# zyhbili/Dual-Space-NeRF

Hardware: AMD Instinct MI355X
Metric: rendered rays/sec (64 samples/ray), 512x512 frame (higher is better)
Workload: dtype split-f16x3 (3 x v_mfma_f32_32x32x16_f16 on hi/lo fp16 operand halves, f32 accumulate: f32-equivalent accuracy - parity bars of the tests: 1e-4 absolute on RGB / acc / weights against the reference; sigma 1e-4 absolute where |sigma| <= 100 and 4e-6 RELATIVE to max|sigma| above (this checkpoint: |sig

## Files before the change

### dual-space-nerf_amd/csrc/dsn_api.hip

```cpp
#include "../../include/dsnerf.h"
#include "dsn_common.h"
#include "dsn_kernels.h"
#include <cstdlib>

#include <stdio.h>
#include <string.h>

static thread_local char g_err[512] = "";

static int dsn_fail(const char* fmt, const char* a = "", long long b = 0) {
    snprintf(g_err, sizeof(g_err), fmt, a, b);
    return 1;
}
static int dsn_check_launch(const char* what) {
    hipError_t e = hipGetLastError();
    if (e != hipSuccess) { snprintf(g_err, sizeof(g_err), "%s: launch failed: %s", what, hipGetErrorString(e)); return 1; }
    return 0;
}
#define DSN_REQUIRE(cond, msg) do { if (!(cond)) return dsn_fail("%s", msg); } while (0)

thread_local int g_dsn_persistent_override = 0;
namespace {
struct DsnShareCus {
    explicit DsnShareCus(bool on) {
// ... 642 lines not shown
        int32_t *counts = nullptr, *outside0 = nullptr;
        dsn_nn_cellmajor_begin(w.nn_small, &counts, &outside0, st);
        dsn_launch_sample_gg(s.xyz, (flags & DSN_SAMPLE_UNIFORM) ? 0 : V, ray_o, ray_d, near, far, R, S, t_vals, jitter, z, nullptr, st,
                             s.nn_world.fine.g, (int32_t*)w.grad, counts, outside0, (int32_t*)w.grad + N);
        if (lazy) dsn_launch_build_nn_visited(s.cent_world, F, s.nn_world, counts, st);
    } else
        dsn_launch_sample_gg(s.xyz, (flags & DSN_SAMPLE_UNIFORM) ? 0 : V, ray_o, ray_d, near, far, R, S, t_vals, jitter, z, nullptr, st);
    if (skip) {
        if (hipMemsetAsync(w.count, 0, DSN_CNT_BYTES, st) != hipSuccess) return dsn_fail("%s", "dsn_render_rays: memset failed");
    }
    if (cellmajor) {
        int32_t* g3 = (int32_t*)w.grad;
        if (!fused_nn) {
            dsn_launch_nn_cellmajor(s.nn_world, nullptr, ray_o, ray_d, z, N, S, g3, w.sort_scratch, g3 + N, w.nn_small, st);
            dsn_launch_warp(s, nullptr, ray_o, ray_d, z, N, S, nullptr, nullptr, nullptr, w.transparent, w.x_c, nullptr, list, cnt, exh, st,
                            g3 + N, skip);
        } else {
            int32_t* outside = nullptr;
            dsn_launch_nn_cellmajor_warp(s.nn_world, ray_o, ray_d, z, N, S, g3, w.sort_scratch, w.nn_small, s.face_world, s.face_canon,
                                         w.transparent, w.x_c, list, cnt, skip, &outside, st, true, lazy);
            dsn_launch_warp(s, nullptr, ray_o, ray_d, z, N, S, nullptr, nullptr, nullptr, w.transparent, w.x_c, nullptr, list, cnt, exh, st,
                            nullptr, skip, g3, outside);
        }
    } else
        dsn_launch_warp(s, nullptr, ray_o, ray_d, z, N, S, nullptr, nullptr, nullptr, w.transparent, w.x_c, nullptr, list, cnt, exh, st,
                        nullptr, skip);
    if (skip) {
        if (hipMemsetAsync(w.sigma, 0, sizeof(float) * N, st) != hipSuccess)
            return dsn_fail("%s", "dsn_render_rays: memset failed");
    }
    }
    if (do_field) {
    int32_t* const fcnt = skip ? w.count + DSN_CNT_FLAGGED : nullptr;
    if (flags & DSN_FIELD_FP32)
        dsn_launch_field((const float*)packed, s.frame, w.x_c, N, list, cnt, w.sigma, w.essence, w.grad, st);
    else if (skip && (flags & DSN_EARLY_STOP)) {
        const bool screen = (flags & DSN_DENSITY_SCREEN) != 0;
        const bool audit = screen && (flags & DSN_SCREEN_AUDIT);
        int32_t* pcnt = w.count + DSN_CNT_POS;
        dsn_launch_slice_bucket(w.active, w.count + DSN_CNT_ACTIVE, N, S, R, bounds, K, w.slices, w.count + DSN_CNT_SLICE, st);
        dsn_launch_slice_T_init(w.T, R, st);
        static const bool adv_env_ray = [] { const char* e = getenv("DSN_STOP_ADVANCE"); return !(e && e[0] == 'l'); }();
        const bool adv_per_ray = adv_env_ray || custom_schedule;
        const float* scal = (const float*)packed + OFF_SCAL;
        for (int k = 0; k < K; ++k) {
            const int s0 = bounds[k], s1 = bounds[k + 1];
            const int64_t Nk = (int64_t)R * (s1 - s0);
            const int32_t* sl = w.slices + (int64_t)R * s0;
            const int32_t* sc = w.count + DSN_CNT_SLICE + k;
            if (k > 0) {
                int32_t* acnt = w.count + DSN_CNT_ALIVE_K + k;
                if (adv_per_ray) dsn_launch_advance_T(w.sigma, w.transparent, z, ray_d, R, S, bounds[k - 1], s0, k, w.T, st);
                dsn_launch_slice_alive(sl, sc, Nk, S, L, k, w.T, w.sigma, w.transparent, z, ray_d, scal, w.alive, acnt, w.count + DSN_CNT_STOP, st,
                                       adv_per_ray);
                sl = w.alive;
                sc = acnt;
            }
            if (screen) {
                int32_t* kcnt = w.count + DSN_CNT_KEEP_K + k;
                dsn_launch_screen16((const float*)packed, s.frame, w.x_c, Nk, sl, sc, w.sigma, w.keep, kcnt, nullptr, nullptr, st,
                                    audit ? w.audit : nullptr, audit ? w.count + DSN_CNT_AUDIT : nullptr, w.audit_cap);
                sl = w.keep;
                sc = kcnt;
            }
            dsn_launch_field16_fwd((const float*)packed, s.frame, w.x_c, Nk, sl, sc, w.sigma, w.essence, w.masks, w.pos, pcnt, st,
                                   w.rec_cap, fcnt);
            (void)s0;
        }
        float* wq = w.n_w;
        dsn_launch_composite(nullptr, w.sigma, w.transparent, z, ray_d, nullptr, R, S, nullptr, nullptr, nullptr, wq, nullptr, st);
        int32_t* sel = w.alive;
        int32_t* lit = w.slices;
        dsn_launch_cull_lit(w.pos, pcnt, N, w.rec_cap, wq, w.sigma, S, scal, sel, w.count + DSN_CNT_SEL, lit, w.count + DSN_CNT_LIT,
                            w.count + DSN_CNT_STOP + 1, w.colour, st);
        dsn_launch_field16_bwd((const float*)packed, s.frame, w.x_c, N, w.pos, pcnt, w.grad, w.masks, st, w.sigma, w.rec_cap, sel,
                               w.count + DSN_CNT_SEL, fcnt);
        if (w.rec_cap < N)
            dsn_launch_field16_from((const float*)packed, s.frame, w.x_c, N, w.pos, pcnt, w.rec_cap, w.sigma, w.essence, w.grad, st, fcnt);
        dsn_launch_field_fix((const float*)packed, s.frame, w.x_c, N, w.pos, pcnt, w.sigma, w.essence, w.grad, st, fcnt);
        if (audit) dsn_launch_screen_audit(w.audit, w.count + DSN_CNT_AUDIT, w.audit_cap, w.sigma, w.count + DSN_CNT_AUDIT + 4, st);
        list = lit;
        cnt = w.count + DSN_CNT_LIT;
    } else if (skip) {
        int32_t* pcnt = w.count + DSN_CNT_POS;
        const bool screen = (flags & DSN_DENSITY_SCREEN) != 0;
        const bool audit = screen && (flags & DSN_SCREEN_AUDIT);
        if (screen) {
            int32_t* kcnt = w.count + DSN_CNT_KEEP;
            dsn_launch_screen16((const float*)packed, s.frame, w.x_c, N, list, cnt, w.sigma, w.keep, kcnt, nullptr, nullptr, st,
                                audit ? w.audit : nullptr, audit ? w.count + DSN_CNT_AUDIT : nullptr, w.audit_cap);
            list = w.keep;
            cnt = kcnt;
        }
        dsn_launch_field16_fwd((const float*)packed, s.frame, w.x_c, N, list, cnt, w.sigma, w.essence, w.masks, w.pos, pcnt, st,
                               w.rec_cap, fcnt);
        dsn_launch_field16_bwd((const float*)packed, s.frame, w.x_c, N, w.pos, pcnt, w.grad, w.masks, st, w.sigma, w.rec_cap, nullptr, nullptr,
                               fcnt);
        list = w.pos;
        cnt = pcnt;
        if (w.rec_cap < N)
            dsn_launch_field16_from((const float*)packed, s.frame, w.x_c, N, list, cnt, w.rec_cap, w.sigma, w.essence, w.grad, st, fcnt);
        dsn_launch_field_fix((const float*)packed, s.frame, w.x_c, N, list, cnt, w.sigma, w.essence, w.grad, st, fcnt);
        if (audit) dsn_launch_screen_audit(w.audit, w.count + DSN_CNT_AUDIT, w.audit_cap, w.sigma, w.count + DSN_CNT_AUDIT + 4, st);
    } else {
        dsn_launch_field16((const float*)packed, s.frame, w.x_c, N, list, cnt, w.sigma, w.essence, w.grad, st);
        dsn_launch_field_fix((const float*)packed, s.frame, w.x_c, N, list, cnt, w.sigma, w.essence, w.grad, st);
    }
    }
    if (!(flags & DSN_FIELD_FP32) && skip) {
        if (flags & DSN_EARLY_STOP) { list = w.slices; cnt = w.count + DSN_CNT_LIT; }
        else { list = w.pos; cnt = w.count + DSN_CNT_POS; }
    }
    if (do_shade && sweep) {
    int32_t n_sh = 0;
    if (hipMemcpyAsync(&n_sh, cnt, sizeof(int32_t), hipMemcpyDeviceToHost, st) != hipSuccess || hipStreamSynchronize(st) != hipSuccess)
        return dsn_fail("%s", "dsn_render_rays_lights: reading the shading list's length failed");
    const size_t per_light = sizeof(float) * 3 * (size_t)n_sh;
    const int G = per_light == 0 ? sweep->n_lights : (int)std::min<size_t>((size_t)sweep->n_lights, sweep->scratch_bytes / per_light);
    if (G < 1)
        return dsn_fail("dsn_render_rays_lights: light_scratch is too small%s: one light's colours need %lld bytes "
                        "(dsn_render_lights_scratch_bytes)", "", (long long)per_light);
    int32_t* slot = w.alive;
    if (!dsn_composite_multi_supported(S, z, w.sigma, out_weights, slot, w.transparent))
        return dsn_fail("%s", "dsn_render_rays_lights: unaligned arrays for the 16-lane compositor");
    dsn_launch_normal(s, w.x_c, w.grad, N, list, cnt, nullptr, w.n_w, exh, st);
    if (hipMemsetAsync(slot, 0xff, sizeof(int32_t) * (size_t)N, st) != hipSuccess)
        return dsn_fail("%s", "dsn_render_rays_lights: memset failed");
    dsn_launch_slot_map(list, cnt, n_sh, slot, st);
// ... 111 lines not shown
```

### dual-space-nerf_amd/csrc/dsn_field16.hip

```cpp
#include "dsn_common.h"
#include "dsn_kernels.h"

typedef float f32x16 __attribute__((ext_vector_type(16)));
typedef _Float16 half8 __attribute__((ext_vector_type(8)));
#define MFMA16(a, b, c) __builtin_amdgcn_mfma_f32_32x32x16_f16((a), (b), (c), 0, 0, 0)

#if !defined(DSN_EXPERIMENTS) && (defined(F16_ABL) || defined(F16_SABL) || defined(F16_TIMING) || defined(F16_TRAIN_ABL))
#error "F16_ABL / F16_SABL / F16_TIMING are experiment switches (wrong results / debug counters): build with -DDSN_EXPERIMENTS"
#endif
#ifndef F16_SINCOS_OCML
#define F16_SINCOS_OCML 0
#endif
#ifndef F16_FENCE
#define F16_FENCE 0
#endif
#ifndef F16_SGB
#define F16_SGB 1
#endif
#ifndef F16_SGB_VALU
#define F16_SGB_VALU 4
#endif
#ifndef F16_SGB_DS
#define F16_SGB_DS 0
#endif
#ifndef F16_MIX
#define F16_MIX 1
#endif
#ifndef F16_PIPE_LATE
#define F16_PIPE_LATE 1
#endif
#ifndef F16_ABL
#define F16_ABL 0
#endif
#ifndef F16_NEXT_POINT
#define F16_NEXT_POINT 1
#endif
#ifndef F16_DMA_SPREAD
#define F16_DMA_SPREAD 1
#endif
#ifndef F16_BIAS_AHEAD
#define F16_BIAS_AHEAD 1
#endif
#ifndef F16_TIMING
#define F16_TIMING 0
#endif
#ifndef F16_PREFETCH
#define F16_PREFETCH 1
#endif

#define F16_THREADS 256
#if defined(DSN_EXPERIMENTS) && defined(F16_TRAIN_ABL) && (F16_TRAIN_ABL & 32)
#define F16_ST_M(m) (1024 * (m))
#else
#define F16_ST_M(m) (32 * (m))
#endif
#define F16_CHUNK 8
#define F16_RING_SLOTS (2 * F16_CHUNK)
#define F16_NCHUNK (DSN_STREAM_BLOCKS / F16_CHUNK)
#define F16_RANGE 65000.0f
#define F16_GSCALE 0.015625f
#define F16_GUNSCALE 64.0f

#if F16_TIMING
__device__ unsigned long long g_f16_timing[16];
#define F16_STAMP(i) do { if (MODE == F16_FWD) { asm volatile("s_waitcnt vmcnt(0) lgkmcnt(0)" ::: "memory"); tstamp[i] = __builtin_readcyclecounter(); rstamp[i] = wall_clock64(); } } while (0)
extern "C" __attribute__((visibility("default"))) int dsn_debug_timing(unsigned long long* out16, int reset) {
    if (out16 && hipMemcpyFromSymbol(out16, HIP_SYMBOL(g_f16_timing), sizeof(unsigned long long) * 16) != hipSuccess) return 1;
    if (reset) { unsigned long long z[16] = {0}; if (hipMemcpyToSymbol(HIP_SYMBOL(g_f16_timing), z, sizeof(z)) != hipSuccess) return 1; }
    return 0;
}
#else
#define F16_STAMP(i) do { } while (0)
#endif
struct W16 {
    const char* g;
    char* ring;
    unsigned ring_off;
    int wave;
    int nchunk = F16_NCHUNK;
    bool spread = F16_DMA_SPREAD != 0;
    half8 h0, l0, h1, l1;
};

#ifndef F16_POS_OFFS
#define F16_POS_OFFS 0
#endif
__device__ __forceinline__ void w16_stage(const W16& w, int c) {
    const char* src = w.g + (size_t)c * 32768;
    const unsigned dst = w.ring_off + (c & 1) * 32768 + w.wave * 8192 + 4096;
#if F16_POS_OFFS
    asm volatile("s_mov_b32 m0, %1\n\ts_nop 0\n\t"
                 "global_load_lds_dwordx4 %0, off\n\tglobal_load_lds_dwordx4 %0, off offset:1024\n\t"
                 "global_load_lds_dwordx4 %0, off offset:2048\n\tglobal_load_lds_dwordx4 %0, off offset:3072"
                 : : "v"(src - 4096), "s"(dst - 4096) : "memory", "m0");
    asm volatile("s_mov_b32 m0, %1\n\ts_nop 0\n\t"
                 "global_load_lds_dwordx4 %0, off\n\tglobal_load_lds_dwordx4 %0, off offset:1024\n\t"
                 "global_load_lds_dwordx4 %0, off offset:2048\n\tglobal_load_lds_dwordx4 %0, off offset:3072"
                 : : "v"(src), "s"(dst) : "memory", "m0");
    return;
#endif
    asm volatile("s_mov_b32 m0, %1\n\ts_nop 0\n\t"
                 "global_load_lds_dwordx4 %0, off offset:-4096\n\tglobal_load_lds_dwordx4 %0, off offset:-3072\n\t"
                 "global_load_lds_dwordx4 %0, off offset:-2048\n\tglobal_load_lds_dwordx4 %0, off offset:-1024\n\t"
                 "global_load_lds_dwordx4 %0, off\n\tglobal_load_lds_dwordx4 %0, off offset:1024\n\t"
                 "global_load_lds_dwordx4 %0, off offset:2048\n\tglobal_load_lds_dwordx4 %0, off offset:3072"
                 : : "v"(src), "s"(dst) : "memory", "m0");
}
template <int I>
__device__ __forceinline__ void w16_stage_part(const W16& w, int c) {
    const char* src = w.g + (size_t)c * 32768;
    const unsigned dst = w.ring_off + (c & 1) * 32768 + w.wave * 8192 + 4096;
#if F16_POS_OFFS
    {
        const int back = I < 2 ? 4096 : 0;
        asm volatile("s_mov_b32 m0, %1\n\ts_nop 0\n\t"
                     "global_load_lds_dwordx4 %0, off offset:%2\n\tglobal_load_lds_dwordx4 %0, off offset:%3"
                     : : "v"(src - back), "s"(dst - back), "n"(2048 * (I & 1)), "n"(2048 * (I & 1) + 1024) : "memory", "m0");
        return;
    }
#endif
    asm volatile("s_mov_b32 m0, %1\n\ts_nop 0\n\t"
                 "global_load_lds_dwordx4 %0, off offset:%2\n\tglobal_load_lds_dwordx4 %0, off offset:%3"
                 : : "v"(src), "s"(dst), "n"(-4096 + 2048 * I), "n"(-3072 + 2048 * I) : "memory", "m0");
}
__device__ __forceinline__ void w16_boundary(const W16& w, int b) {
#if !(F16_ABL & 2)
    asm volatile("s_waitcnt vmcnt(0)" ::: "memory");
#endif
#if !(F16_ABL & 1)
    __syncthreads();
#endif
    const int c = b / F16_CHUNK;
#if !(F16_ABL & 4)
    if (!w.spread && c + 1 < w.nchunk) w16_stage(w, c + 1);
#endif
}
__device__ __forceinline__ void w16_read(const W16& w, int b, int lane, half8& h0, half8& l0, half8& h1, half8& l1) {
    const char* s = w.ring + ((b >> 3) & 1) * 32768 + (b & 7) * 1024 + lane * 16;
    h0 = *reinterpret_cast<const half8*>(s);
    l0 = *reinterpret_cast<const half8*>(s + 8192);
    h1 = *reinterpret_cast<const half8*>(s + 16384);
    l1 = *reinterpret_cast<const half8*>(s + 24576);
}
__device__ __forceinline__ void w16_begin_issue(W16& w, int first_blk) { w16_stage(w, first_blk / F16_CHUNK); }
__device__ __forceinline__ void w16_begin_wait(W16& w, int lane, int first_blk) {
    w16_boundary(w, first_blk);
#if !(F16_ABL & 4)
    if (w.spread && first_blk / F16_CHUNK + 1 < w.nchunk) w16_stage_part<0>(w, first_blk / F16_CHUNK + 1);
#endif
    w16_read(w, first_blk, lane, w.h0, w.l0, w.h1, w.l1);
}
__device__ __forceinline__ void w16_begin(W16& w, int lane, int first_blk) {
    w16_begin_issue(w, first_blk);
    w16_begin_wait(w, lane, first_blk);
}

struct NoHook { __device__ __forceinline__ void operator()(int) const {} };

template <int KB, bool XLS, class Hook = NoHook>
__device__ __forceinline__ void dense16(W16& w, int& blk, int lane, const half8 (&xh)[KB][2], const half8 (&xl)[KB][2],
                                        f32x16& accM, f32x16& accC, Hook&& hook = NoHook()) {
#pragma unroll
    for (int kb = 0; kb < KB; ++kb) {
#if F16_PREFETCH
        half8 n0 = w.h0, m0 = w.l0, n1 = w.h1, m1 = w.l1;
        if (blk + 1 < DSN_STREAM_BLOCKS) {
            if (((blk + 1) & (F16_CHUNK - 1)) == 0) w16_boundary(w, blk + 1);
#if !(F16_ABL & 4)
            if (w.spread) {
                const int pos = (blk + 1) & (F16_CHUNK - 1), cn = (blk + 1) / F16_CHUNK + 1;
                if (cn < w.nchunk) {
                    if (pos == 0) w16_stage_part<0>(w, cn);
                    if (pos == 1) w16_stage_part<1>(w, cn);
                    if (pos == 2) w16_stage_part<2>(w, cn);
                    if (pos == 3) w16_stage_part<3>(w, cn);
                }
            }
#endif
            w16_read(w, blk + 1, lane, n0, m0, n1, m1);
        }
#else
        if (blk > 0) {
            if ((blk & (F16_CHUNK - 1)) == 0) w16_boundary(w, blk);
            w16_read(w, blk, lane, w.h0, w.l0, w.h1, w.l1);
        }
#endif
        if (XLS) {
            accM = MFMA16(w.h0, xh[kb][0], accM);
            accC = MFMA16(w.h0, xl[kb][0], accC);
            accC = MFMA16(w.l0, xh[kb][0], accC);
            accM = MFMA16(w.h1, xh[kb][1], accM);
            accC = MFMA16(w.h1, xl[kb][1], accC);
            accC = MFMA16(w.l1, xh[kb][1], accC);
        } else {
            accM = MFMA16(w.h0, xh[kb][0], accM);
            accC = MFMA16(w.l0, xh[kb][0], accC);
            accM = MFMA16(w.h0, xl[kb][0], accM);
            accC = MFMA16(w.h1, xh[kb][1], accC);
            accM = MFMA16(w.l1, xh[kb][1], accM);
            accC = MFMA16(w.h1, xl[kb][1], accC);
        }
#if !(F16_ABL & 8)
        hook(kb);
#endif
// ... 281 lines not shown
    }
}
template <bool ST = false>
__device__ __forceinline__ void layer16_bwd(W16& w, int& blk, int lane, const half8 (&xh)[8][2],
                                            const half8 (&xl)[8][2], half8 (&yh)[8][2], half8 (&yl)[8][2],
                                            const uint32_t (&mk)[4], float& ovf, float* st = nullptr, float stscale = F16_GUNSCALE) {
    f32x16 pM = zero16(), pC = zero16();
    uint32_t dummy = 0;
#pragma unroll
    for (int m = 0; m < 8; ++m) {
        f32x16 aM = zero16(), aC = zero16();
        const uint32_t mw = m > 0 ? ((mk[(m - 1) >> 1] >> (16 * ((m - 1) & 1))) & 0xffffu) : 0u;
        if (m == 0) dense16<8, true>(w, blk, lane, xh, xl, aM, aC);
        else dense16<8, true>(w, blk, lane, xh, xl, aM, aC, [&](int kb) { epi_slice<false, ST>(pM, pC, kb, mw, dummy, yh[m - 1], yl[m - 1], ovf, (ST && st) ? st + F16_ST_M(m - 1) : nullptr, stscale); });
        pM = aM; pC = aC;
    }
    const uint32_t mw = (mk[3] >> 16) & 0xffffu;
#pragma unroll
    for (int kb = 0; kb < 8; ++kb) epi_slice<false, ST>(pM, pC, kb, mw, dummy, yh[7], yl[7], ovf, (ST && st) ? st + F16_ST_M(7) : nullptr, stscale);
}

#define F16_FULL 0
#define F16_FWD 1
#define F16_BWD 2
#define F16_TRAIN 3
#define F16_FIRST_BWD_BLOCK (OFF_L6T / DSN_BLK)
template <int MODE>
__global__ void __launch_bounds__(F16_THREADS, 1)
k_field16(const float* __restrict__ packed, const DsnFrameState* __restrict__ fs, const float* __restrict__ x_c,
          int64_t N, const int32_t* __restrict__ active_list, const int32_t* __restrict__ active_count,
          float* __restrict__ sigma, float* __restrict__ essence, float* __restrict__ grad,
          uint4* __restrict__ masks, int32_t* __restrict__ pos_list, int32_t* __restrict__ pos_count,
          float* __restrict__ tr_h, float* __restrict__ tr_a, float* __restrict__ tr_rr, int64_t slot_base, int64_t rec_cap,
          const int32_t* __restrict__ sel, int32_t* __restrict__ flag_count) {
    constexpr bool ST = MODE == F16_TRAIN;
    __shared__ __attribute__((aligned(16))) char ring[F16_RING_SLOTS * 4096];
    __shared__ uint32_t s_mask[7][4][F16_THREADS];
    __shared__ __attribute__((aligned(16))) float s_vec[256 + 2304 + 8];
    __shared__ __attribute__((aligned(16))) half8 s_pe[8][F16_THREADS];
    __shared__ int s_app[8];
#ifndef F16_SHARE_SIMD
    DSN_OWN_SIMD();
#endif
    const int tid0 = threadIdx.x;
    const int lane0 = threadIdx.x & 63;
    const int wave = __builtin_amdgcn_readfirstlane(threadIdx.x >> 6);
    int64_t count = (active_list ? (int64_t)(*active_count) : N) - slot_base;
    if (MODE == F16_BWD && count > rec_cap) count = rec_cap;
    const int64_t ntiles = (count + 127) / 128;
    if ((int64_t)blockIdx.x >= ntiles) return;
    for (int i = tid0; i < 256 + 2304 + 8; i += F16_THREADS)
        s_vec[i] = i < 256 ? fs->bias0[i] : (i < 2560 ? packed[OFF_B1 + (i - 256)] : packed[OFF_SCAL + (i - 2560)]);
    for (int i = tid0; i < 256 + (OFF_WDEN - OFF_B1); i += F16_THREADS) s_vec[i] *= F16_FWD_SCALE;
    const float* const v_bias0 = s_vec;
    const float* const v_b1 = s_vec + 256;
    const float* const v_brgb1 = s_vec + 256 + (OFF_BRGB1 - OFF_B1);
    const float* const v_wden = s_vec + 256 + (OFF_WDEN - OFF_B1);
    const float* const v_wrgb3 = s_vec + 256 + (OFF_WRGB3 - OFF_B1);
    const float* const v_scal = s_vec + 2560;
    W16 w;
    w.g = reinterpret_cast<const char*>(packed + OFF16_BASE) + wave * 8192 + 4096 + lane0 * 16;
    w.ring = ring;
    w.ring_off = (unsigned)(uintptr_t)(__attribute__((address_space(3))) char*)ring;
    w.wave = wave;
    if (MODE == F16_FWD) w.nchunk = F16_FIRST_BWD_BLOCK / F16_CHUNK;
    if (MODE == F16_TRAIN) w.spread = false;
    auto tile_point = [&](int64_t t, bool& ok, int64_t& ls) -> int64_t {
        int64_t sl = (t * 4 + wave) * 32 + (lane0 & 31);
        ok = sl < count;
        if (!ok) sl = count - 1;
        ls = sel ? (int64_t)sel[sl] : slot_base + sl;
        return active_list ? (int64_t)active_list[ls] : ls;
    };
    bool valid_n;
    int64_t lslot_n;
    int64_t pt_n = tile_point(blockIdx.x, valid_n, lslot_n);
    float xn[3] = {x_c[3 * pt_n], x_c[3 * pt_n + 1], x_c[3 * pt_n + 2]};
  for (int64_t tile = blockIdx.x; tile < ntiles; tile += gridDim.x) {
    int tid = tid0, lane = lane0;
    asm volatile("" : "+v"(tid), "+v"(lane), "+v"(w.g));
    const int half = lane >> 5;
#if F16_TIMING
    unsigned long long tstamp[6], rstamp[6];
#endif
    F16_STAMP(0);
    w16_begin_issue(w, MODE == F16_BWD ? F16_FIRST_BWD_BLOCK : 0);
#if !F16_NEXT_POINT
    if (tile != (int64_t)blockIdx.x) { pt_n = tile_point(tile, valid_n, lslot_n); xn[0] = x_c[3 * pt_n]; xn[1] = x_c[3 * pt_n + 1]; xn[2] = x_c[3 * pt_n + 2]; }
#endif
    const bool valid = valid_n;
    const int64_t lslot = lslot_n, pt = pt_n;
    const float xa[3] = {xn[0], xn[1], xn[2]};
    const bool more = F16_NEXT_POINT && MODE != F16_TRAIN && tile + gridDim.x < ntiles;
    if (more) pt_n = tile_point(tile + gridDim.x, valid_n, lslot_n);
#define NEXT_POINT() do { if (more) { xn[0] = x_c[3 * pt_n]; xn[1] = x_c[3 * pt_n + 1]; xn[2] = x_c[3 * pt_n + 2]; } } while (0)
    w16_begin_wait(w, lane, MODE == F16_BWD ? F16_FIRST_BWD_BLOCK : 0);
    int blk = MODE == F16_BWD ? F16_FIRST_BWD_BLOCK : 0;
    F16_STAMP(1);

#define MK_STORE(L, mk) { s_mask[L][0][tid] = mk[0]; s_mask[L][1][tid] = mk[1]; s_mask[L][2][tid] = mk[2]; s_mask[L][3][tid] = mk[3]; }
#define MK_LOAD(L, mk) { mk[0] = s_mask[L][0][tid]; mk[1] = s_mask[L][1][tid]; mk[2] = s_mask[L][2][tid]; mk[3] = s_mask[L][3][tid]; }
    uint32_t mk[4];
    half8 ah[8][2], al[8][2], bh[8][2], bl[8][2];
    float ovf = 0.0f;
    uint4* mrec = masks ? masks + ((size_t)(MODE == F16_BWD ? lslot : pt) * 2 + half) * 7 : nullptr;
    const int64_t tr_ls = N * 256;
#if defined(DSN_EXPERIMENTS) && defined(F16_TRAIN_ABL)
    const int64_t pt_st = (F16_TRAIN_ABL & 8) ? (pt & 4095) : ((F16_TRAIN_ABL & 16) ? (pt & 255) : pt);
    const int64_t sl_st = (tile * 4 + wave) * 32 + (lane & 31);
    const int64_t row_off = (F16_TRAIN_ABL & 32) ? (sl_st >> 5) * 8192 + (sl_st & 31) * 32 : pt_st * 256;
    float* const th = ST && valid && !(F16_TRAIN_ABL & 1) ? tr_h + row_off + 4 * half : nullptr;
    float* const ta = ST && valid && !(F16_TRAIN_ABL & 2) ? tr_a + row_off + 4 * half : nullptr;
#else
    float* const th = ST && valid ? tr_h + pt * 256 + 4 * half : nullptr;
    float* const ta = ST && valid ? tr_a + pt * 256 + 4 * half : nullptr;
#endif

  if (MODE != F16_BWD) {
    half8 ph[2][2], pl[2][2];
    {
        f32x16 pe[2];
#pragma unroll
        for (int t = 0; t < 30; ++t) {
            float s, c;
#if F16_SINCOS_OCML
            sincosf(xa[t % 3] * (float)(1 << (t / 3)), &s, &c);
#else
            dsn_sincos(xa[t % 3] * (float)(1 << (t / 3)), s, c);
#endif
// ... 44 lines not shown
        }
        f32x16 v = unscale16(aM, aC);
        const uint32_t bits = relu_bits16(v);
        if (m & 1) mk[m >> 1] |= bits << 16; else mk[m >> 1] = bits;
        if (ST) store16(th ? th + 4 * tr_ls + F16_ST_M(m) : nullptr, v, 1.0f);
        track16(ovf, v);
        split16<false>(v, ah[m], al[m]);
    }
    MK_STORE(4, mk)
    layer16_fwd<ST>(w, blk, lane, v_b1 + 4 * 256, ah, al, bh, bl, mk, ovf, th ? th + 5 * tr_ls : nullptr); MK_STORE(5, mk)
    float sg_part = 0.0f;
#pragma unroll
    for (int m = 0; m < 8; ++m) {
        f32x16 aM = rows16(v_b1 + 5 * 256, m, half), aC = zero16();
        dense16<8, false>(w, blk, lane, bh, bl, aM, aC);
        f32x16 v = unscale16(aM, aC);
        const uint32_t bits = relu_bits16(v);
        if (m & 1) mk[m >> 1] |= bits << 16; else mk[m >> 1] = bits;
        if (ST) store16(th ? th + 6 * tr_ls + F16_ST_M(m) : nullptr, v, 1.0f);
        const f32x16 wd = rows16(v_wden, m, half);
#pragma unroll
        for (int r = 0; r < 16; ++r) sg_part = fmaf(wd[r], v[r], sg_part);
        track16(ovf, v);
        split16<false>(v, ah[m], al[m]);
    }
#endif
    F16_STAMP(3);
    sg_part += __shfl_xor(sg_part, 32);
    const float sg = sg_part + v_scal[0];
    const bool flag_fwd = !(fmaxf(ovf, __shfl_xor(ovf, 32)) < F16_RANGE);
    if (valid && half == 0) sigma[pt] = flag_fwd ? dsn_nan_flag() : sg;
    if (MODE != F16_TRAIN && flag_fwd && valid && half == 0 && flag_count) atomicAdd(flag_count, 1);
    bool write_rec = ST && valid;
    if (MODE == F16_FWD) {
        const bool pos = valid && half == 0 && (sg > 0.0f || flag_fwd);
        const unsigned long long bm = __ballot(pos);
        const int cnt = __popcll(bm);
        if (lane == 0) s_app[wave] = cnt;
        __syncthreads();
        if (tid == 0) {
            const int tot = s_app[0] + s_app[1] + s_app[2] + s_app[3];
            s_app[4] = tot ? atomicAdd(pos_count, tot) : 0;
        }
        __syncthreads();
        int base = s_app[4];
        for (int k = 0; k < wave; ++k) base += s_app[k];
        const int my = base + __popcll(bm & ((1ull << lane) - 1ull));
        if (pos) pos_list[my] = (int32_t)pt;
        const int rslot = __shfl(my, lane & 31);
        write_rec = ((bm >> (lane & 31)) & 1ull) != 0 && (int64_t)rslot < rec_cap;
        mrec = masks + ((size_t)rslot * 2 + half) * 7;
    }
    if (MODE == F16_FWD || MODE == F16_TRAIN) {
        MK_STORE(6, mk)
        if (write_rec) {
#pragma unroll
            for (int L = 0; L < 7; ++L)
                mrec[L] = make_uint4(s_mask[L][0][tid], s_mask[L][1][tid], s_mask[L][2][tid], s_mask[L][3][tid]);
        }
    }
    {
        float e0 = 0.f, e1 = 0.f, e2 = 0.f;
#pragma unroll
        for (int m = 0; m < 4; ++m) {
            f32x16 aM = rows16(v_brgb1, m, half), aC = zero16();
            dense16<8, false>(w, blk, lane, ah, al, aM, aC);
            const f32x16 v = unscale16(aM, aC);
            const f32x16 w0 = rows16(v_wrgb3 + 0 * 128, m, half);
            const f32x16 w1 = rows16(v_wrgb3 + 1 * 128, m, half);
            const f32x16 w2 = rows16(v_wrgb3 + 2 * 128, m, half);
            if (ST && valid) {
                f32x16 xr;
#pragma unroll
                for (int r = 0; r < 16; ++r) xr[r] = fmaxf(v[r], 0.0f);
                store16(tr_rr + pt * 128 + 4 * half + 32 * m, xr, 1.0f);
            }
#pragma unroll
            for (int r = 0; r < 16; ++r) {
                const float x = fmaxf(v[r], 0.0f);
                e0 = fmaf(w0[r], x, e0); e1 = fmaf(w1[r], x, e1); e2 = fmaf(w2[r], x, e2);
            }
        }
        e0 += __shfl_xor(e0, 32); e1 += __shfl_xor(e1, 32); e2 += __shfl_xor(e2, 32);
        if (valid && half == 0) {
            essence[3 * pt + 0] = e0 + v_scal[1];
            essence[3 * pt + 1] = e1 + v_scal[2];
            essence[3 * pt + 2] = e2 + v_scal[3];
        }
    }

#if F16_TIMING
    F16_STAMP(4);
    if (MODE == F16_FWD && tid == 0) {
        for (int i = 0; i < 4; ++i) { atomicAdd(&g_f16_timing[i], tstamp[i + 1] - tstamp[i]); atomicAdd(&g_f16_timing[8 + i], rstamp[i + 1] - rstamp[i]); }
        atomicAdd(&g_f16_timing[7], 1ull);
    }
#endif
    if (MODE == F16_FWD) { __syncthreads(); continue; }
  } else {
#pragma unroll
    for (int L = 0; L < 7; ++L) {
        const uint4 q = mrec[L];
        s_mask[L][0][tid] = q.x; s_mask[L][1][tid] = q.y; s_mask[L][2][tid] = q.z; s_mask[L][3][tid] = q.w;
    }
    MK_LOAD(6, mk)
  }

#pragma unroll
    for (int m = 0; m < 8; ++m) {
        f32x16 g = rows16(v_wden, m, half);
#pragma unroll
        for (int r = 0; r < 16; ++r) g[r] *= F16_GSCALE;
        mask16(g, (mk[m >> 1] >> (16 * (m & 1))) & 0xffffu);
        if (ST) store16(ta ? ta + 6 * tr_ls + F16_ST_M(m) : nullptr, g, F16_GUNSCALE);
        split16<true>(g, ah[m], al[m]);
    }
    MK_LOAD(5, mk) layer16_bwd<ST>(w, blk, lane, ah, al, bh, bl, mk, ovf, ta ? ta + 5 * tr_ls : nullptr);
    if (MODE == F16_BWD) NEXT_POINT();
    MK_LOAD(4, mk) layer16_bwd<ST>(w, blk, lane, bh, bl, ah, al, mk, ovf, ta ? ta + 4 * tr_ls : nullptr);
    MK_LOAD(3, mk)
    f32x16 dpe[2];
#pragma unroll
    for (int m = 0; m < 8; ++m) {
        f32x16 aM = zero16(), aC = zero16();
        dense16<8, true>(w, blk, lane, ah, al, aM, aC);
        f32x16 v = fold16(aM, aC);
        mask16(v, (mk[m >> 1] >> (16 * (m & 1))) & 0xffffu);
        if (ST) store16(ta ? ta + 3 * tr_ls + F16_ST_M(m) : nullptr, v, F16_GUNSCALE);
        track16(ovf, v);
        split16<true>(v, bh[m], bl[m]);
    }
// ... 15 lines not shown
        for (int r = 0; r < 16; ++r) dpe[b][r] += v[r];
    }

    {
        float xb[3] = {xa[0], xa[1], xa[2]};
        asm volatile("" : "+v"(xb[0]), "+v"(xb[1]), "+v"(xb[2]));
        float g[3] = {0.f, 0.f, 0.f};
#pragma unroll
        for (int t = 0; t < 30; ++t) {
            const int j = t / 3, a = t % 3;
            float s, c;
#if F16_SINCOS_OCML
            sincosf(xb[a] * (float)(1 << j), &s, &c);
#else
            dsn_sincos(xb[a] * (float)(1 << j), s, c);
#endif
            const float d = dpe[t >> 4][t & 15];
            const float term = (d * (half ? s : c)) * (float)(1 << j);
            g[a] += half ? -term : term;
        }
        const float i30 = dpe[1][14], i31 = dpe[1][15];
        if (half) g[1] += i30; else { g[0] += i30; g[2] += i31; }
        g[0] += __shfl_xor(g[0], 32); g[1] += __shfl_xor(g[1], 32); g[2] += __shfl_xor(g[2], 32);
        if (valid && half == 0) {
            grad[3 * pt] = g[0] * F16_GUNSCALE; grad[3 * pt + 1] = g[1] * F16_GUNSCALE; grad[3 * pt + 2] = g[2] * F16_GUNSCALE;
        }
    }
    const bool flagged = !(fmaxf(ovf, __shfl_xor(ovf, 32)) < F16_RANGE);
    if (flagged && valid && half == 0) {
        if (MODE == F16_TRAIN) { if (pos_count) atomicAdd(pos_count, 1); }
        else { sigma[pt] = dsn_nan_flag(); if (flag_count) atomicAdd(flag_count, 1); }
    }
    if (MODE == F16_TRAIN) break;
    __syncthreads();
  }
}

void dsn_launch_field16(const float* packed, const DsnFrameState* fs, const float* x_c, int64_t N,
                        const int32_t* active_list, const int32_t* active_count, float* sigma, float* essence,
                        float* grad, hipStream_t st, int32_t* flag_count) {
    int64_t blocks = (N + 127) / 128;
    if (blocks == 0) return;
    hipLaunchKernelGGL(k_field16<F16_FULL>, dim3((unsigned)std::min<int64_t>(blocks, dsn_cu_count())), dim3(F16_THREADS), 0, st, packed, fs, x_c, N,
                       active_list, active_count, sigma, essence, grad, (uint4*)nullptr, (int32_t*)nullptr,
                       (int32_t*)nullptr, (float*)nullptr, (float*)nullptr, (float*)nullptr, (int64_t)0, (int64_t)0, (const int32_t*)nullptr,
                       flag_count);
}
void dsn_launch_field16_from(const float* packed, const DsnFrameState* fs, const float* x_c, int64_t N, const int32_t* list,
                             const int32_t* count, int64_t slot_base, float* sigma, float* essence, float* grad, hipStream_t st,
                             int32_t* flag_count) {
    int64_t blocks = (N - slot_base + 127) / 128;
    if (blocks <= 0) return;
    hipLaunchKernelGGL(k_field16<F16_FULL>, dim3((unsigned)std::min<int64_t>(blocks, dsn_cu_count())), dim3(F16_THREADS), 0, st, packed, fs, x_c, N, list, count, sigma,
                       essence, grad, (uint4*)nullptr, (int32_t*)nullptr, (int32_t*)nullptr, (float*)nullptr, (float*)nullptr,
                       (float*)nullptr, slot_base, (int64_t)0, (const int32_t*)nullptr, flag_count);
}
void dsn_launch_field16_train(const float* packed, const DsnFrameState* fs, const float* x_c, int64_t N, float* sigma,
                              float* essence, float* grad, float* tr_h, float* tr_a, float* tr_rr, void* masks, hipStream_t st,
                              int32_t* range_count, const int32_t* row_list, const int32_t* row_count) {
    int64_t blocks = (N + 127) / 128;
    if (blocks == 0) return;
    hipLaunchKernelGGL(k_field16<F16_TRAIN>, dim3((unsigned)blocks), dim3(F16_THREADS), 0, st, packed, fs, x_c, N,
                       row_list, row_count, sigma, essence, grad, (uint4*)masks, (int32_t*)nullptr,
                       range_count, tr_h, tr_a, tr_rr, (int64_t)0, N, (const int32_t*)nullptr, (int32_t*)nullptr);
}
void dsn_launch_field16_fwd(const float* packed, const DsnFrameState* fs, const float* x_c, int64_t N,
                            const int32_t* active_list, const int32_t* active_count, float* sigma, float* essence,
                            void* masks, int32_t* pos_list, int32_t* pos_count, hipStream_t st, int64_t rec_cap, int32_t* flag_count) {
    int64_t blocks = (N + 127) / 128;
    if (blocks == 0) return;
    hipLaunchKernelGGL(k_field16<F16_FWD>, dim3((unsigned)std::min<int64_t>(blocks, dsn_cu_count())), dim3(F16_THREADS), 0, st, packed, fs, x_c, N,
                       active_list, active_count, sigma, essence, (float*)nullptr, (uint4*)masks, pos_list, pos_count,
                       (float*)nullptr, (float*)nullptr, (float*)nullptr, (int64_t)0, rec_cap, (const int32_t*)nullptr, flag_count);
}
void dsn_launch_field16_bwd(const float* packed, const DsnFrameState* fs, const float* x_c, int64_t N,
                            const int32_t* pos_list, const int32_t* pos_count, float* grad, const void* masks,
                            hipStream_t st, float* sigma, int64_t rec_cap, const int32_t* sel, const int32_t* sel_count,
                            int32_t* flag_count) {
    int64_t blocks = ((rec_cap < N ? rec_cap : N) + 127) / 128;
    if (blocks == 0) return;
    hipLaunchKernelGGL(k_field16<F16_BWD>, dim3((unsigned)std::min<int64_t>(blocks, dsn_cu_count())), dim3(F16_THREADS), 0, st, packed, fs, x_c, N,
                       pos_list, sel ? sel_count : pos_count, sigma, (float*)nullptr, grad, (uint4*)masks, (int32_t*)nullptr,
                       (int32_t*)nullptr, (float*)nullptr, (float*)nullptr, (float*)nullptr, (int64_t)0, rec_cap, sel, flag_count);
}

__device__ __forceinline__ void epi_slice_tan(const f32x16& pM, const f32x16& pC, int kb, uint32_t mword, half8 (&yh)[2],
                                              half8 (&yl)[2], float* st, float stscale, float& ovf, float* keep = nullptr) {
    float vv[2];
#pragma unroll
    for (int e = 0; e < 2; ++e) {
        const int r = 2 * kb + e;
        const float v = dsn_keep_active((pM[r] + pC[r]) * F16_FWD_INV, mword, r);
        vv[e] = v;
        const _Float16 hi = (_Float16)v;
        yh[r >> 3][r & 7] = hi;
        yl[r >> 3][r & 7] = (_Float16)fmaf((float)hi, -1.0f, v);
    }
    asm("v_max3_f32 %0, %0, |%1|, |%2|" : "+v"(ovf) : "v"(vv[0]), "v"(vv[1]));
#if defined(DSN_EXPERIMENTS) && defined(F16_TRAIN_ABL) && (F16_TRAIN_ABL & 256)
    if (kb == 7) {
        float o[16];
#pragma unroll
        for (int r = 0; r < 16; ++r) o[r] = dsn_keep_active((pM[r] + pC[r]) * F16_FWD_INV, mword, r) * stscale;
        store16_lines_emul(st, o);
        return;
    }
#endif
    if (keep && kb == 7) {
#pragma unroll
        for (int r = 0; r < 16; ++r) keep[r] = dsn_keep_active((pM[r] + pC[r]) * F16_FWD_INV, mword, r) * stscale;
        return;
    }
    if (st && kb == 7) {
#pragma unroll
        for (int q = 0; q < 4; ++q) {
            float o[4];
// ... 1155 lines not shown
```

### dual-space-nerf_amd/csrc/dsn_kernels.h

```cpp
#pragma once
#include "dsn_common.h"

#include <algorithm>
#include <cstdlib>
extern thread_local int g_dsn_persistent_override;
inline int dsn_cu_count_raw();
inline int dsn_cu_count() { return g_dsn_persistent_override > 0 ? g_dsn_persistent_override : dsn_cu_count_raw(); }
inline int dsn_cu_count_raw() {
    static const int n = [] {
        int dev = 0, v = 0;
        if (hipGetDevice(&dev) != hipSuccess || hipDeviceGetAttribute(&v, hipDeviceAttributeMultiprocessorCount, dev) != hipSuccess || v <= 0) v = 256;
        const char* e = getenv("DSN_PERSISTENT_GROUPS");
        if (e && atoi(e) > 0) v = atoi(e);
        return v;
    }();
    return n;
}

void dsn_launch_face_setup(const float* verts, const int32_t* faces, int F, DsnFaceRec* recs, float4* cent,
                           hipStream_t st);
void dsn_launch_pose_setup(const float* packed, const float* poses, int frame_idx, int zero_code,
                           const float* light_shift, const float* rot, const float* rot_center, DsnFrameState* fs,
                           hipStream_t st, const float* pose_feat16 = nullptr);
void dsn_launch_sample_gg(const float* xyz, int V, const float* ray_o, const float* ray_d, float* near, float* far,
// ... 2 lines not shown
                          int32_t* cls_counts = nullptr, int32_t* cls_outside = nullptr, int32_t* cls_rank_of = nullptr);
void dsn_nn_cellmajor_begin(void* small, int32_t** counts, int32_t** outside, hipStream_t st);
void dsn_launch_warp(const DsnSceneView& s, const float* pts, const float* ray_o, const float* ray_d,
                     const float* z_vals, int64_t N, int S, int32_t* face_idx, float* uv, float* h,
                     uint8_t* transparent, float* x_c, float* ray_d_can, int32_t* active_list, int32_t* active_count,
                     bool exhaustive, hipStream_t st, const int32_t* nn_pre = nullptr, bool lazy_canon = false,
                     const int32_t* only_cell_of = nullptr, const int32_t* only_count = nullptr);
size_t dsn_nn_sort_scratch_size(int64_t N);
void dsn_launch_nn_cellmajor_coarse(const DsnNNView& v, const float4* cent, const float* pts, const uint8_t* live, int64_t N,
                                    int32_t* cell_of, void* sorted, int32_t* nn, void* small, hipStream_t st, void* keys8N = nullptr, int F = 0,
                                    int32_t* wave_scratch = nullptr, int64_t wave_scratch_ints = 0);
void dsn_launch_nn_cellmajor(const DsnNNView& v, const float* pts, const float* ray_o, const float* ray_d, const float* z_vals,
                             int64_t N, int S, int32_t* cell_of, void* sorted, int32_t* nn, void* small, hipStream_t st);
void dsn_launch_nn_cellmajor_warp(const DsnNNView& v, const float* ray_o, const float* ray_d, const float* z_vals, int64_t N, int S,
                                  int32_t* cell_of, void* sorted, void* small, const DsnFaceRec* face_world, const DsnFaceRec* face_canon,
                                  uint8_t* transparent, float* x_c, int32_t* active_list, int32_t* active_count, bool lazy_canon,
                                  int32_t** outside, hipStream_t st, bool classified = false, bool lazy_call = false);
void dsn_launch_lbs_warp(const DsnSceneView& s, const float* pts, int64_t N, const float* smpl_w, const float* A, int bw_type,
                         int32_t* face_idx, float* weights, uint8_t* transparent, float* pts_zero, bool exhaustive, hipStream_t st);
void dsn_launch_normal(const DsnSceneView& s, const float* x_c, const float* grad, int64_t N,
                       const int32_t* active_list, const int32_t* active_count, int32_t* face_idx_canon, float* n_w,
                       bool exhaustive, hipStream_t st, const int32_t* nn_far = nullptr);
void dsn_launch_build_nn(const float4* cent, int F, const DsnNNView& nn, float pad_fine, float pad_coarse, hipStream_t st,
                         bool fine_only = false, bool dense_fine = false, bool lazy = false);
void dsn_launch_build_nn_visited(const float4* cent, int F, const DsnNNView& nn, const int32_t* visited, hipStream_t st);
void dsn_launch_build_nn_complete(const float4* cent, int F, const DsnNNView& nn, hipStream_t st);
void dsn_launch_composite(const float* colour, const float* sigma, const uint8_t* transparent, const float* z_vals,
                          const float* ray_d, const float* noise, int R, int S, float* rgb_map, float* disp_map,
                          float* acc_map, float* weights, float* depth_map, hipStream_t st, bool lazy_colour = false,
                          int32_t* colour_max = nullptr);
void dsn_launch_field16_fwd(const float* packed, const DsnFrameState* fs, const float* x_c, int64_t N,
                            const int32_t* active_list, const int32_t* active_count, float* sigma, float* essence,
                            void* masks, int32_t* pos_list, int32_t* pos_count, hipStream_t st, int64_t rec_cap,
                            int32_t* flag_count = nullptr);
void dsn_launch_field16_from(const float* packed, const DsnFrameState* fs, const float* x_c, int64_t N, const int32_t* list,
                             const int32_t* count, int64_t slot_base, float* sigma, float* essence, float* grad, hipStream_t st,
                             int32_t* flag_count = nullptr);
void dsn_launch_field16_bwd(const float* packed, const DsnFrameState* fs, const float* x_c, int64_t N,
                            const int32_t* pos_list, const int32_t* pos_count, float* grad, const void* masks,
                            hipStream_t st, float* sigma, int64_t rec_cap, const int32_t* sel = nullptr,
                            const int32_t* sel_count = nullptr, int32_t* flag_count = nullptr);
void dsn_launch_screen16(const float* packed, const DsnFrameState* fs, const float* x_c, int64_t N, const int32_t* active_list,
                         const int32_t* active_count, float* sigma, int32_t* keep_list, int32_t* keep_count, float* dbg_sigma,
                         float* dbg_s1, hipStream_t st, int32_t* audit_list = nullptr, int32_t* audit_count = nullptr,
                         int audit_cap = 0);
void dsn_launch_screen_audit(const int32_t* audit_list, const int32_t* audit_count, int audit_cap, const float* sigma, int32_t* out,
                             hipStream_t st);
size_t dsn_calibrate_workspace_size(int64_t n);
void dsn_launch_calibrate_screen(const DsnSceneView& s, float* packed, int64_t n, void* workspace, float* out4, hipStream_t st,
                                 const float* frame_x_c = nullptr, const int32_t* frame_list = nullptr,
                                 const int32_t* frame_count = nullptr);
void dsn_launch_set_screen_margin(float* packed, float margin, hipStream_t st);
void dsn_launch_set_packed_scalar(float* packed, int word, float v, hipStream_t st);
void dsn_launch_light16(const float* packed, const DsnFrameState* fs, const float* n_w, const float* x_w,
                        const float* ray_o, const float* ray_d, const float* z_vals, const float* essence, int64_t N,
                        int S, const int32_t* active_list, const int32_t* active_count, float* colour, hipStream_t st,
                        float* tr_hl1 = nullptr, float* tr_hl2 = nullptr, float* tr_pre = nullptr);
void dsn_launch_light16_multi(const float* packed, const DsnLightEdit* lights, int G, const float* n_w, const float* ray_o, const float* ray_d,
                              const float* z_vals, const float* essence, int64_t max_count, int S, const int32_t* list,
                              const int32_t* list_count, float* colours, hipStream_t st);
void dsn_launch_slot_map(const int32_t* list, const int32_t* count, int64_t max_count, int32_t* slot, hipStream_t st);
bool dsn_composite_multi_supported(int S, const void* z_vals, const void* sigma, const void* weights, const void* slot_of,
                                   const void* transparent);
void dsn_launch_composite_multi(const int32_t* slot_of, const float* colours, int64_t n_shaded, int G, const float* sigma,
                                const uint8_t* transparent, const float* z_vals, const float* ray_d, int R, int S, float* rgb_maps,
                                float* disp_map, float* acc_map, float* weights, float* depth_map, int32_t* colour_max, hipStream_t st);
void dsn_launch_camera_rays(const double* K, const double* R, const double* T, const double* bounds, int H, int W,
// ... 66 lines not shown
```

Before: 28.76 million.

## Keep weight ring streaming across persistent tiles and skip essence for empty tiles

Persistent field16 forward and backward kernels now wrap the weight-chunk staging ring into the next tile. Each new tile starts with its first chunk already staged, which removes the per-tile __syncthreads and the cold-start load. The backward pass uses the s_pe buffer as an extra slot for its first chunk. The forward pass also skips the essence (RGB) head when a tile has no positive-sigma points, controlled by an env var that defaults to lazy. This adds tricky cross-tile LDS reuse and synchronisation, with risk of races or stale data.

```diff
diff --git a/dual-space-nerf_amd/csrc/dsn_api.hip b/dual-space-nerf_amd/csrc/dsn_api.hip
--- a/dual-space-nerf_amd/csrc/dsn_api.hip
+++ b/dual-space-nerf_amd/csrc/dsn_api.hip
@@ -698,6 +698,8 @@
     }
     if (do_field) {
     int32_t* const fcnt = skip ? w.count + DSN_CNT_FLAGGED : nullptr;
+    const char* eager_env = getenv("DSN_EAGER_ESSENCE");
+    const bool lazy_essence = !(eager_env && eager_env[0] == '1');
     if (flags & DSN_FIELD_FP32)
         dsn_launch_field((const float*)packed, s.frame, w.x_c, N, list, cnt, w.sigma, w.essence, w.grad, st);
     else if (skip && (flags & DSN_EARLY_STOP)) {
@@ -730,7 +732,7 @@
                 sc = kcnt;
             }
             dsn_launch_field16_fwd((const float*)packed, s.frame, w.x_c, Nk, sl, sc, w.sigma, w.essence, w.masks, w.pos, pcnt, st,
-                                   w.rec_cap, fcnt);
+                                   w.rec_cap, fcnt, lazy_essence);
             (void)s0;
         }
         float* wq = w.n_w;
@@ -759,7 +761,7 @@
             cnt = kcnt;
         }
         dsn_launch_field16_fwd((const float*)packed, s.frame, w.x_c, N, list, cnt, w.sigma, w.essence, w.masks, w.pos, pcnt, st,
-                               w.rec_cap, fcnt);
+                               w.rec_cap, fcnt, lazy_essence);
         dsn_launch_field16_bwd((const float*)packed, s.frame, w.x_c, N, w.pos, pcnt, w.grad, w.masks, st, w.sigma, w.rec_cap, nullptr, nullptr,
                                fcnt);
         list = w.pos;
diff --git a/dual-space-nerf_amd/csrc/dsn_field16.hip b/dual-space-nerf_amd/csrc/dsn_field16.hip
--- a/dual-space-nerf_amd/csrc/dsn_field16.hip
+++ b/dual-space-nerf_amd/csrc/dsn_field16.hip
@@ -46,6 +46,12 @@
 #endif
 #ifndef F16_PREFETCH
 #define F16_PREFETCH 1
+#endif
+#ifndef F16_RING_CONT
+#define F16_RING_CONT 1
+#endif
+#ifndef F16_SKIP_RGB
+#define F16_SKIP_RGB 1
 #endif
 
 #define F16_THREADS 256
@@ -80,14 +86,24 @@
     int nchunk = F16_NCHUNK;
     bool spread = F16_DMA_SPREAD != 0;
     half8 h0, l0, h1, l1;
+    int first = 0;
+    int wrap = 0;
+    bool alt = false;
+    const char* alt_ptr = nullptr;
+    unsigned alt_off = 0;
 };
+__device__ __forceinline__ int w16_src_chunk(const W16& w, int c) { return c < w.nchunk ? c : c - w.nchunk + w.first; }
+__device__ __forceinline__ unsigned w16_slot_off(const W16& w, int c) {
+    return (w.alt && w16_src_chunk(w, c) == w.first) ? w.alt_off : w.ring_off + (c & 1) * 32768;
+}
+__device__ __forceinline__ bool w16_staged(const W16& w, int c) { return c < w.nchunk || c < w.nchunk + w.wrap; }
 
 #ifndef F16_POS_OFFS
 #define F16_POS_OFFS 0
 #endif
 __device__ __forceinline__ void w16_stage(const W16& w, int c) {
-    const char* src = w.g + (size_t)c * 32768;
-    const unsigned dst = w.ring_off + (c & 1) * 32768 + w.wave * 8192 + 4096;
+    const char* src = w.g + (size_t)w16_src_chunk(w, c) * 32768;
+    const unsigned dst = w16_slot_off(w, c) + w.wave * 8192 + 4096;
 #if F16_POS_OFFS
     asm volatile("s_mov_b32 m0, %1\n\ts_nop 0\n\t"
                  "global_load_lds_dwordx4 %0, off\n\tglobal_load_lds_dwordx4 %0, off offset:1024\n\t"
@@ -108,8 +124,8 @@
 }
 template <int I>
 __device__ __forceinline__ void w16_stage_part(const W16& w, int c) {
-    const char* src = w.g + (size_t)c * 32768;
-    const unsigned dst = w.ring_off + (c & 1) * 32768 + w.wave * 8192 + 4096;
+    const char* src = w.g + (size_t)w16_src_chunk(w, c) * 32768;
+    const unsigned dst = w16_slot_off(w, c) + w.wave * 8192 + 4096;
 #if F16_POS_OFFS
     {
         const int back = I < 2 ? 4096 : 0;
@@ -132,11 +148,11 @@
 #endif
     const int c = b / F16_CHUNK;
 #if !(F16_ABL & 4)
-    if (!w.spread && c + 1 < w.nchunk) w16_stage(w, c + 1);
+    if (!w.spread && w16_staged(w, c + 1)) w16_stage(w, c + 1);
 #endif
 }
 __device__ __forceinline__ void w16_read(const W16& w, int b, int lane, half8& h0, half8& l0, half8& h1, half8& l1) {
-    const char* s = w.ring + ((b >> 3) & 1) * 32768 + (b & 7) * 1024 + lane * 16;
+    const char* s = ((w.alt && (b >> 3) == w.first) ? w.alt_ptr : w.ring + ((b >> 3) & 1) * 32768) + (b & 7) * 1024 + lane * 16;
     h0 = *reinterpret_cast<const half8*>(s);
     l0 = *reinterpret_cast<const half8*>(s + 8192);
     h1 = *reinterpret_cast<const half8*>(s + 16384);
@@ -169,7 +185,7 @@
 #if !(F16_ABL & 4)
             if (w.spread) {
                 const int pos = (blk + 1) & (F16_CHUNK - 1), cn = (blk + 1) / F16_CHUNK + 1;
-                if (cn < w.nchunk) {
+                if (w16_staged(w, cn)) {
                     if (pos == 0) w16_stage_part<0>(w, cn);
                     if (pos == 1) w16_stage_part<1>(w, cn);
                     if (pos == 2) w16_stage_part<2>(w, cn);
@@ -517,7 +533,7 @@
           float* __restrict__ sigma, float* __restrict__ essence, float* __restrict__ grad,
           uint4* __restrict__ masks, int32_t* __restrict__ pos_list, int32_t* __restrict__ pos_count,
           float* __restrict__ tr_h, float* __restrict__ tr_a, float* __restrict__ tr_rr, int64_t slot_base, int64_t rec_cap,
-          const int32_t* __restrict__ sel, int32_t* __restrict__ flag_count) {
+          const int32_t* __restrict__ sel, int32_t* __restrict__ flag_count, bool lazy_essence) {
     constexpr bool ST = MODE == F16_TRAIN;
     __shared__ __attribute__((aligned(16))) char ring[F16_RING_SLOTS * 4096];
     __shared__ uint32_t s_mask[7][4][F16_THREADS];
@@ -550,6 +566,14 @@
     w.wave = wave;
     if (MODE == F16_FWD) w.nchunk = F16_FIRST_BWD_BLOCK / F16_CHUNK;
     if (MODE == F16_TRAIN) w.spread = false;
+    constexpr bool CONT = F16_RING_CONT && (MODE == F16_FWD || MODE == F16_BWD);
+    if (MODE == F16_BWD) w.first = F16_FIRST_BWD_BLOCK / F16_CHUNK;
+    if (CONT && MODE == F16_BWD) {
+        w.alt = true;
+        w.alt_ptr = reinterpret_cast<const char*>(&s_pe[0][0]);
+        w.alt_off = (unsigned)(uintptr_t)(__attribute__((address_space(3))) char*)(char*)&s_pe[0][0];
+    }
+    int ring_state = 0;
     auto tile_point = [&](int64_t t, bool& ok, int64_t& ls) -> int64_t {
         int64_t sl = (t * 4 + wave) * 32 + (lane0 & 31);
         ok = sl < count;
@@ -569,7 +593,8 @@
     unsigned long long tstamp[6], rstamp[6];
 #endif
     F16_STAMP(0);
-    w16_begin_issue(w, MODE == F16_BWD ? F16_FIRST_BWD_BLOCK : 0);
+    if (ring_state == 0) w16_begin_issue(w, MODE == F16_BWD ? F16_FIRST_BWD_BLOCK : 0);
+    w.wrap = CONT && tile + gridDim.x < ntiles ? (MODE == F16_FWD ? 2 : 1) : 0;
 #if !F16_NEXT_POINT
     if (tile != (int64_t)blockIdx.x) { pt_n = tile_point(tile, valid_n, lslot_n); xn[0] = x_c[3 * pt_n]; xn[1] = x_c[3 * pt_n + 1]; xn[2] = x_c[3 * pt_n + 2]; }
 #endif
@@ -579,7 +604,8 @@
     const bool more = F16_NEXT_POINT && MODE != F16_TRAIN && tile + gridDim.x < ntiles;
     if (more) pt_n = tile_point(tile + gridDim.x, valid_n, lslot_n);
 #define NEXT_POINT() do { if (more) { xn[0] = x_c[3 * pt_n]; xn[1] = x_c[3 * pt_n + 1]; xn[2] = x_c[3 * pt_n + 2]; } } while (0)
-    w16_begin_wait(w, lane, MODE == F16_BWD ? F16_FIRST_BWD_BLOCK : 0);
+    if (CONT && MODE == F16_FWD && ring_state == 2) w16_read(w, 0, lane, w.h0, w.l0, w.h1, w.l1);
+    else w16_begin_wait(w, lane, MODE == F16_BWD ? F16_FIRST_BWD_BLOCK : 0);
     int blk = MODE == F16_BWD ? F16_FIRST_BWD_BLOCK : 0;
     F16_STAMP(1);
 
@@ -690,6 +716,7 @@
     if (valid && half == 0) sigma[pt] = flag_fwd ? dsn_nan_flag() : sg;
     if (MODE != F16_TRAIN && flag_fwd && valid && half == 0 && flag_count) atomicAdd(flag_count, 1);
     bool write_rec = ST && valid;
+    int tile_pos = 1;
     if (MODE == F16_FWD) {
         const bool pos = valid && half == 0 && (sg > 0.0f || flag_fwd);
         const unsigned long long bm = __ballot(pos);
@@ -701,6 +728,7 @@
             s_app[4] = tot ? atomicAdd(pos_count, tot) : 0;
         }
         __syncthreads();
+        tile_pos = __builtin_amdgcn_readfirstlane(s_app[0] + s_app[1] + s_app[2] + s_app[3]);
         int base = s_app[4];
         for (int k = 0; k < wave; ++k) base += s_app[k];
         const int my = base + __popcll(bm & ((1ull << lane) - 1ull));
@@ -717,6 +745,17 @@
                 mrec[L] = make_uint4(s_mask[L][0][tid], s_mask[L][1][tid], s_mask[L][2][tid], s_mask[L][3][tid]);
         }
     }
+#if F16_TIMING
+    if (MODE == F16_FWD && tid == 0 && tile_pos == 0) atomicAdd(&g_f16_timing[5], 1ull);
+#endif
+#if F16_SKIP_RGB
+    if (MODE == F16_FWD && lazy_essence && tile_pos == 0) {
+        asm volatile("s_waitcnt vmcnt(0)" ::: "memory");
+        if (CONT && w.wrap) { w16_begin_issue(w, 0); ring_state = 1; }
+        continue;
+    }
+#endif
+    F16_STAMP(4);
     {
         float e0 = 0.f, e1 = 0.f, e2 = 0.f;
 #pragma unroll
@@ -748,13 +787,17 @@
     }
 
 #if F16_TIMING
-    F16_STAMP(4);
+    F16_STAMP(5);
     if (MODE == F16_FWD && tid == 0) {
-        for (int i = 0; i < 4; ++i) { atomicAdd(&g_f16_timing[i], tstamp[i + 1] - tstamp[i]); atomicAdd(&g_f16_timing[8 + i], rstamp[i + 1] - rstamp[i]); }
+        for (int i = 0; i < 5; ++i) { atomicAdd(&g_f16_timing[i], tstamp[i + 1] - tstamp[i]); atomicAdd(&g_f16_timing[8 + i], rstamp[i + 1] - rstamp[i]); }
         atomicAdd(&g_f16_timing[7], 1ull);
     }
 #endif
-    if (MODE == F16_FWD) { __syncthreads(); continue; }
+    if (MODE == F16_FWD) {
+        if (CONT) ring_state = 2;
+        else __syncthreads();
+        continue;
+    }
   } else {
 #pragma unroll
     for (int L = 0; L < 7; ++L) {
@@ -836,7 +879,8 @@
         else { sigma[pt] = dsn_nan_flag(); if (flag_count) atomicAdd(flag_count, 1); }
     }
     if (MODE == F16_TRAIN) break;
-    __syncthreads();
+    if (CONT) ring_state = 1;
+    else __syncthreads();
   }
 }
 
@@ -848,7 +892,7 @@
     hipLaunchKernelGGL(k_field16<F16_FULL>, dim3((unsigned)std::min<int64_t>(blocks, dsn_cu_count())), dim3(F16_THREADS), 0, st, packed, fs, x_c, N,
                        active_list, active_count, sigma, essence, grad, (uint4*)nullptr, (int32_t*)nullptr,
                        (int32_t*)nullptr, (float*)nullptr, (float*)nullptr, (float*)nullptr, (int64_t)0, (int64_t)0, (const int32_t*)nullptr,
-                       flag_count);
+                       flag_count, false);
 }
 void dsn_launch_field16_from(const float* packed, const DsnFrameState* fs, const float* x_c, int64_t N, const int32_t* list,
                              const int32_t* count, int64_t slot_base, float* sigma, float* essence, float* grad, hipStream_t st,
@@ -857,7 +901,7 @@
     if (blocks <= 0) return;
     hipLaunchKernelGGL(k_field16<F16_FULL>, dim3((unsigned)std::min<int64_t>(blocks, dsn_cu_count())), dim3(F16_THREADS), 0, st, packed, fs, x_c, N, list, count, sigma,
                        essence, grad, (uint4*)nullptr, (int32_t*)nullptr, (int32_t*)nullptr, (float*)nullptr, (float*)nullptr,
-                       (float*)nullptr, slot_base, (int64_t)0, (const int32_t*)nullptr, flag_count);
+                       (float*)nullptr, slot_base, (int64_t)0, (const int32_t*)nullptr, flag_count, false);
 }
 void dsn_launch_field16_train(const float* packed, const DsnFrameState* fs, const float* x_c, int64_t N, float* sigma,
                               float* essence, float* grad, float* tr_h, float* tr_a, float* tr_rr, void* masks, hipStream_t st,
@@ -866,16 +910,18 @@
     if (blocks == 0) return;
     hipLaunchKernelGGL(k_field16<F16_TRAIN>, dim3((unsigned)blocks), dim3(F16_THREADS), 0, st, packed, fs, x_c, N,
                        row_list, row_count, sigma, essence, grad, (uint4*)masks, (int32_t*)nullptr,
-                       range_count, tr_h, tr_a, tr_rr, (int64_t)0, N, (const int32_t*)nullptr, (int32_t*)nullptr);
+                       range_count, tr_h, tr_a, tr_rr, (int64_t)0, N, (const int32_t*)nullptr, (int32_t*)nullptr, false);
 }
 void dsn_launch_field16_fwd(const float* packed, const DsnFrameState* fs, const float* x_c, int64_t N,
                             const int32_t* active_list, const int32_t* active_count, float* sigma, float* essence,
-                            void* masks, int32_t* pos_list, int32_t* pos_count, hipStream_t st, int64_t rec_cap, int32_t* flag_count) {
+                            void* masks, int32_t* pos_list, int32_t* pos_count, hipStream_t st, int64_t rec_cap, int32_t* flag_count,
+                            bool lazy_essence) {
     int64_t blocks = (N + 127) / 128;
     if (blocks == 0) return;
     hipLaunchKernelGGL(k_field16<F16_FWD>, dim3((unsigned)std::min<int64_t>(blocks, dsn_cu_count())), dim3(F16_THREADS), 0, st, packed, fs, x_c, N,
                        active_list, active_count, sigma, essence, (float*)nullptr, (uint4*)masks, pos_list, pos_count,
-                       (float*)nullptr, (float*)nullptr, (float*)nullptr, (int64_t)0, rec_cap, (const int32_t*)nullptr, flag_count);
+                       (float*)nullptr, (float*)nullptr, (float*)nullptr, (int64_t)0, rec_cap, (const int32_t*)nullptr, flag_count,
+                       lazy_essence);
 }
 void dsn_launch_field16_bwd(const float* packed, const DsnFrameState* fs, const float* x_c, int64_t N,
                             const int32_t* pos_list, const int32_t* pos_count, float* grad, const void* masks,
@@ -885,7 +931,7 @@
     if (blocks == 0) return;
     hipLaunchKernelGGL(k_field16<F16_BWD>, dim3((unsigned)std::min<int64_t>(blocks, dsn_cu_count())), dim3(F16_THREADS), 0, st, packed, fs, x_c, N,
                        pos_list, sel ? sel_count : pos_count, sigma, (float*)nullptr, grad, (uint4*)masks, (int32_t*)nullptr,
-                       (int32_t*)nullptr, (float*)nullptr, (float*)nullptr, (float*)nullptr, (int64_t)0, rec_cap, sel, flag_count);
+                       (int32_t*)nullptr, (float*)nullptr, (float*)nullptr, (float*)nullptr, (int64_t)0, rec_cap, sel, flag_count, false);
 }
 
 __device__ __forceinline__ void epi_slice_tan(const f32x16& pM, const f32x16& pC, int kb, uint32_t mword, half8 (&yh)[2],
diff --git a/dual-space-nerf_amd/csrc/dsn_kernels.h b/dual-space-nerf_amd/csrc/dsn_kernels.h
--- a/dual-space-nerf_amd/csrc/dsn_kernels.h
+++ b/dual-space-nerf_amd/csrc/dsn_kernels.h
@@ -58,7 +58,7 @@
 void dsn_launch_field16_fwd(const float* packed, const DsnFrameState* fs, const float* x_c, int64_t N,
                             const int32_t* active_list, const int32_t* active_count, float* sigma, float* essence,
                             void* masks, int32_t* pos_list, int32_t* pos_count, hipStream_t st, int64_t rec_cap,
-                            int32_t* flag_count = nullptr);
+                            int32_t* flag_count = nullptr, bool lazy_essence = false);
 void dsn_launch_field16_from(const float* packed, const DsnFrameState* fs, const float* x_c, int64_t N, const int32_t* list,
                              const int32_t* count, int64_t slot_base, float* sigma, float* essence, float* grad, hipStream_t st,
                              int32_t* flag_count = nullptr);
```

After: 29.02 million (median of 6 runs). No clear change (+0.9%).
